# Ushio/MassiveVoxelRayTracing

Measured on AMD Instinct MI355X. Metric: Mrays/sec (primary+secondary) at 1920x1080, 64 spp, higher is better.
Workload: dtype f32; 1 GPU; xyzrgb_dragon stand-in 2048^3 SVO (procedural, pinned by tests/test_scenes.py), wavefront path trace 1920x1080, 183 steps of 16 spp rendered as 64-spp frames (frame buffer cleared + device synchronised per frame), 8 bounces + IBL shadow rays; voxels=18903401, dag_nodes=643656, triangles=1102122, parallelism=1 GPU, device= (gfx950:sramecc+:xnack-, 256 CUs)

## Files before the change

massivevoxelraytracing_amd/csrc/kernels_rt.hip:

```cpp
#include <stdlib.h>

#include <type_traits>

#include "launch.h"
#include "traverse_stream.h"

#define WAVE 64
#define CBLOCK 256

MVRT_DI uint32_t laneId() { return __builtin_amdgcn_mbcnt_hi( ~0u, __builtin_amdgcn_mbcnt_lo( ~0u, 0u ) ); }

MVRT_DI unsigned long long waveSum( unsigned long long v )
{
	for( int o = 32; o > 0; o >>= 1 ) v += __shfl_down( v, o, WAVE );
	return v;
}

static int numCUs();

#define STREAM_WAVES_PER_CU 32

struct BatchIO
{
	const float *rox, *roy, *roz, *rdx, *rdy, *rdz;
// ... 421 lines not shown

template <class T>
MVRT_DI const __attribute__( ( address_space( 4 ) ) ) T* opaquePtr( const T* p )
{
	asm volatile( "" : "+s"( p ) );
	return (const __attribute__( ( address_space( 4 ) ) ) T*)p;
}

struct PtIO
{
	const PtBuffers* table;
	int setIdx;
	uint32_t n;
	int shadowKind;
	int useHint;
	MVRT_UTIL_COUNTERS
	uint32_t dNormal, dShadow, nHits;
	MVRT_DI int kindOf( uint32_t r, uint32_t* i ) const
	{
		const uint32_t kindSlot = ( r >= n ? 1u : 0u ) + ( r >= 2u * n ? 1u : 0u );
		*i = r - ( kindSlot == 0u ? 0u : ( kindSlot == 1u ? n : 2u * n ) );
		return kindSlot == 0 ? 0 : ( kindSlot == 1 ? ( shadowKind ? 1 : 2 ) : 2 );
	}
	MVRT_DI bool load( uint32_t r, f3* ro, f3* rd, uint32_t* hint ) const
	{
		const __attribute__( ( address_space( 4 ) ) ) PtBuffers& buf = *opaquePtr( table );
		const __attribute__( ( address_space( 4 ) ) ) PathSet& in = buf.set[setIdx];
		uint32_t i;
		const int kind = kindOf( r, &i );
		*ro = mk3( in.rox[i], in.roy[i], in.roz[i] );
		if( useHint ) *hint = in.org[i];
		const float *x0 = in.rdx, *y0 = in.rdy, *z0 = in.rdz, *x1 = buf.sx, *y1 = buf.sy, *z1 = buf.sz, *x2 = buf.ex, *y2 = buf.ey, *z2 = buf.ez;
		const float* const px = kind == 0 ? x0 : ( kind == 1 ? x1 : x2 );
		const float* const py = kind == 0 ? y0 : ( kind == 1 ? y1 : y2 );
		const float* const pz = kind == 0 ? z0 : ( kind == 1 ? z1 : z2 );
		*rd = mk3( px[i], py[i], pz[i] );
		return kind == 1;
	}
	MVRT_DI void store( uint32_t r, const StreamHit& h, bool )
	{
		const __attribute__( ( address_space( 4 ) ) ) PtBuffers& buf = *opaquePtr( table );
		uint32_t i;
		const int kind = kindOf( r, &i );
		const bool isHit = h.t != MVRT_MAXF;
		if( kind == 0 )
		{
			buf.hitT[i] = h.t;
			buf.hitPath[i] = h.path;
			buf.hitN[i] = (uint8_t)h.nMajor;
			if( isHit ) atomicAdd( &buf.blockCount[i / CBLOCK], 1u );
		}
		else if( kind == 1 )
		{
			buf.hitS[i] = isHit ? 1 : 0;
		}
		else
		{
			buf.hitE[i] = isHit ? 1 : 0;
			buf.hitEPath[i] = h.path;
		}
		dShadow += kind == 1 ? h.descents : 0u;
		dNormal += kind == 1 ? 0u : h.descents;
		nHits += ( kind != 1 && isHit ) ? 1u : 0u;
	}
};
template <int FL>
__global__ void __launch_bounds__( 64, MVRT_WAVES_OF( FL ) ) kPtTraceStream( PtParams P, TraceWorkspace ws, int stage, int setIdx, int nKinds, int shadowKind, uint32_t chunk,
																			uint32_t raysPerLane, uint32_t minWaves )
{
	PtIO io;
	io.table = P.buf.selfDev;
	io.setIdx = setIdx;
	io.n = P.buf.liveCount[stage];
	io.shadowKind = shadowKind;
	io.useHint = ( FL == 0 && stage > 0 && P.useHints ) ? 1 : 0;
	io.dNormal = io.dShadow = io.nHits = 0;
	const uint64_t total = (uint64_t)io.n * nKinds;
	uint64_t nWaves = gridDim.x;
	if( raysPerLane )
	{
		uint64_t wantWaves = total / ( 64ull * raysPerLane ) + 1;
		if( wantWaves < minWaves ) wantWaves = minWaves;
		if( blockIdx.x >= wantWaves ) return;
		if( wantWaves < nWaves ) nWaves = wantWaves;
	}
	uint64_t c = total / ( nWaves * 4 );
	c = ( c + 63 ) / 64 * 64;
	if( c < 64 ) c = 64;
	if( c > chunk ) c = chunk;
	traceStream<FL>( makeTraceCore( P.svo ), io, total, P.buf.cursors + stage, (uint32_t)c, ws );
	unsigned long long dN = waveSum( (unsigned long long)io.dNormal ), dS = waveSum( (unsigned long long)io.dShadow ), nH = waveSum( (unsigned long long)io.nHits );
#ifdef MVRT_UTIL_STATS
	if( threadIdx.x == 0 )
	{
		atomicAdd( &P.buf.stats[8 + 0], io.utilIters );
		atomicAdd( &P.buf.stats[8 + 1], io.utilActive );
		atomicAdd( &P.buf.stats[8 + 2], io.utilTailIters );
		atomicAdd( &P.buf.stats[8 + 3], io.utilTailActive );
		atomicAdd( &P.buf.stats[12], io.utilRefillClocks );
		atomicAdd( &P.buf.stats[13], io.utilTotalClocks );
		atomicMax( &P.buf.stats[16 + stage], io.utilTailIters );
		atomicAdd( &P.buf.stats[32 + stage], 1ull );
	}
	{
		unsigned long long m = io.utilMaxRayIters;
		for( int o = 32; o > 0; o >>= 1 )
		{
			const unsigned long long t = __shfl_xor( m, o );
			m = t > m ? t : m;
		}
		if( threadIdx.x == 0 ) atomicMax( &P.buf.stats[48 + stage], m );
	}
#endif
	if( threadIdx.x == 0 )
	{
		if( dN ) atomicAdd( &P.buf.stats[2], dN );
		if( dS ) atomicAdd( &P.buf.stats[3], dS );
		if( nH ) atomicAdd( &P.buf.stats[4], nH );
	}
}

MVRT_DI f3 hdriSampleNearest( const HdriDev& h, f3 d, bool isPrimary )
{
	int w = isPrimary ? h.widthPrimary : h.width;
	int hh = isPrimary ? h.heightPrimary : h.height;
	float phi = mvrt_atan2( d.z, d.x ) + MVRT_PI;
	float theta = mvrt_atan2( sqrtf( d.x * d.x + d.z * d.z ), d.y );
	float u = phi / ( MVRT_PI * 2.0f );
	float v = theta / MVRT_PI;
	int x = (int)smin( smax( u * w, 0.0f ), (float)( w - 1.0f ) );
	int y = (int)smin( smax( v * hh, 0.0f ), (float)( hh - 1.0f ) );
	uint64_t index = (uint64_t)y * w + x;
	const float4* px = ( isPrimary && h.pixelsPrimary ) ? h.pixelsPrimary : h.pixels;
	if( !px ) return mk3( 0.0f, 0.0f, 0.0f );
	float4 c = px[index];
	return mk3( c.x, c.y, c.z ) * h.scale;
}
MVRT_DI uint32_t satH( const HdriDev& h, const uint32_t* s, uint32_t x ) { return x == 0 ? 0u : s[h.width * ( h.height - 1 ) + x - 1]; }
MVRT_DI uint32_t satV( const HdriDev& h, const uint32_t* s, uint32_t x, uint32_t y )
{
	if( y == 0 ) return 0u;
	uint32_t s0 = x == 0 ? 0u : s[h.width * ( y - 1 ) + ( x - 1 )];
	uint32_t s1 = s[h.width * ( y - 1 ) + x];
	return s1 - s0;
}
MVRT_DI uint32_t satCount( const HdriDev& h, const uint32_t* s, uint32_t x, uint32_t y )
{
	uint32_t a = ( x == 0 || y == 0 ) ? 0u : s[h.width * ( y - 1 ) + ( x - 1 )];
	uint32_t b = ( y == 0 ) ? 0u : s[h.width * ( y - 1 ) + x];
	uint32_t c = ( x == 0 ) ? 0u : s[h.width * y + ( x - 1 )];
	uint32_t d = s[h.width * y + x];
	return ( d - b ) + ( a - c );
}
MVRT_DI void hdriImportanceSample( const HdriDev& h, f3* dir, f3* L, float* pdf, f3 N, float u0, float u1, float u2, float u3 )
{
	const uint32_t* s = h.sat;
	uint32_t zero = h.zeroTables;
	const float k = 0.8f;
	if( k < N.x ) s = h.sats[0], zero >>= 1;
	else if( N.x < -k ) s = h.sats[1], zero >>= 2;
	else if( k < N.y ) s = h.sats[2], zero >>= 3;
	else if( N.y < -k ) s = h.sats[3], zero >>= 4;
	else if( k < N.z ) s = h.sats[4], zero >>= 5;
	else if( N.z < -k ) s = h.sats[5], zero >>= 6;
	if( zero & 1u )
	{
		*dir = N;
		*L = mk3( 0.0f, 0.0f, 0.0f );
		*pdf = 1.0f;
		return;
	}

	int i = 0, j = h.width;
	while( i < j )
	{
		int m = ( i + j ) / 2;
		float value = (float)satH( h, s, m ) / 4294967296.0f;
		if( value <= u0 ) i = m + 1;
		else j = m;
	}
	uint32_t X = (uint32_t)( i - 1 );
	uint32_t vol = satH( h, s, X + 1 ) - satH( h, s, X );
	i = 0;
	j = h.height;
	while( i < j )
	{
		int m = ( i + j ) / 2;
		float value = (float)satV( h, s, X, m ) / (float)vol;
		if( value <= u1 ) i = m + 1;
		else j = m;
	}
	uint32_t Y = (uint32_t)( i - 1 );
	float pSelection = (float)satCount( h, s, X, Y ) / 4294967296.0f;
	float dTheta = MVRT_PI / (float)h.height;
	float dPhi = 2.0f * MVRT_PI / (float)h.width;
	float theta = Y * dTheta;
	float dH = 2.0f * mvrt_sin( dTheta * 0.5f ) * mvrt_sin( dTheta * 0.5f + theta );
	float sr = dH * dPhi;
	float sY = mixf( mvrt_cos( theta ), mvrt_cos( theta + dTheta ), u2 );
	float phi = dPhi * ( (float)X + u3 ) + MVRT_PI;
	float sX, sZ;
	mvrt_sincos( phi, &sZ, &sX );
	float sinTheta = sqrtf( smax( 1.0f - sY * sY, 0.0f ) );
	*dir = mk3( sX * sinTheta, sY, sZ * sinTheta );
	*pdf = pSelection / sr;
	float4 color = h.pixels[Y * h.width + X];
	*L = mk3( color.x, color.y, color.z ) * h.scale;
}

MVRT_DI f3 sampleLambertian( float a, float b, f3 Ng )
{
	float r = sqrtf( a );
	float theta = b * MVRT_PI * 2.0f;
	float sn, cs;
	mvrt_sincos( theta, &sn, &cs );
	float x = r * cs;
	float y = r * sn;
	float z = sqrtf( smax( 1.0f - a, 0.0f ) );
	const float sign = copysignf( 1.0f, Ng.z );
	const float aa = -1.0f / ( sign + Ng.z );
	const float bb = Ng.x * Ng.y * aa;
	f3 xaxis = mk3( 1.0f + sign * Ng.x * Ng.x * aa, sign * bb, -sign * Ng.x );
	f3 yaxis = mk3( bb, sign + Ng.y * Ng.y * aa, -Ng.y );
	return xaxis * x + yaxis * y + Ng * z;
}

MVRT_DI f3 voxelEmission( const SvoDev& s, uint32_t vIndex, bool withScale )
{
	return rawReflectance( s.attrs[vIndex].y ) * ( withScale ? s.emissionScale : 1.0f );
}

#ifndef MVRT_SHADE_WAVES
#define MVRT_SHADE_WAVES 5
#endif
template <int WAVES, class... ACTIVE>
__global__ void __launch_bounds__( WAVE, WAVES ) kPtShade( PtParams P, int stage, int inSet, ACTIVE... active )
{
	const uint64_t n = P.buf.liveCount[stage];
	const PathSet& in = P.buf.set[inSet];
	const PathSet& out = P.buf.set[inSet ^ 1];
	const bool lastStage = stage >= MVRT_MAX_DEPTH;
	const uint64_t nBlocks = ( n + CBLOCK - 1 ) / CBLOCK;
	for( uint64_t vb = blockIdx.x; vb < nBlocks; vb += gridDim.x )
	{
		uint32_t blockOffset = 0;
		if( !lastStage )
		{
			blockOffset = scanOffset( P.buf.blockCount, P.buf.tileBase, vb );
			if( threadIdx.x == 0 ) P.buf.blockCount[vb] = 0u;
		}
#pragma unroll 1
		for( uint64_t i = vb * CBLOCK + threadIdx.x; i < vb * CBLOCK + CBLOCK; i += WAVE )
		{
			if( i - threadIdx.x >= n ) break;
			const bool valid = i < n;
			bool alive = false;
			uint32_t task = 0, vIndex = 0;
			uint2 attr = make_uint2( 0u, 0u );
			uint64_t hitPath = 0;
			int nMajor = 0;
			float t = MVRT_MAXF;
			f3 ro, rd, T, L;
			if( valid )
			{
				task = in.task[i];
				ro = mk3( in.rox[i], in.roy[i], in.roz[i] );
				rd = mk3( in.rdx[i], in.rdy[i], in.rdz[i] );
				t = P.buf.hitT[i];
				nMajor = P.buf.hitN[i];
				const bool hit = t != MVRT_MAXF;
				hitPath = hit ? P.buf.hitPath[i] : 0ull;
				vIndex = hit ? voxelIndexFromPath( P.svo, hitPath ) : 0u;
				if( hit ) attr = P.svo.attrs[vIndex];
				if( stage == 0 )
				{
					T = mk3( 1.0f, 1.0f, 1.0f );
					L = mk3( 0.0f, 0.0f, 0.0f );
					if( !hit )
					{
						L = L + T * hdriSampleNearest( P.hdri, rd, true );
					}
					else
					{
						L = L + T * rawReflectance( attr.y );
					}
				}
				else
				{
					T = mk3( in.Tx[i], in.Ty[i], in.Tz[i] );
					L = mk3( in.Lx[i], in.Ly[i], in.Lz[i] );
					if( P.hdriEnabled && P.buf.hitS[i] == 0 )
					{
						L = L + mk3( in.nx[i], in.ny[i], in.nz[i] );
					}
					if( stage == 1 && P.extraSamples )
					{
						if( P.buf.hitE[i] )
						{
							const uint32_t ev = voxelIndexFromPath( P.svo, P.buf.hitEPath[i] );
							f3 Le = voxelEmission( P.svo, ev, true );
							L = L + T * Le / (float)( 1 + P.extraSamples );
						}
					}
					if( hit )
					{
						f3 Le = rawReflectance( attr.y ) * P.svo.emissionScale;
						L = L + T * Le * ( stage == 1 ? 1.0f / (float)( 1 + P.extraSamples ) : 1.0f );
					}
				}
				alive = hit && !lastStage;
				if( !alive )
				{
					P.buf.Lsx[task] = L.x;
					P.buf.Lsy[task] = L.y;
					P.buf.Lsz[task] = L.z;
				}
			}
			if( lastStage ) continue;
			const unsigned long long aliveLanes = __ballot( alive );
			const uint32_t rank = __popcll( aliveLanes & ( ( 1ull << threadIdx.x ) - 1ull ) );
			const uint32_t slotBase = blockOffset;
			blockOffset += __popcll( aliveLanes );
			if( alive )
			{
				const uint64_t j = (uint64_t)slotBase + rank;
				uint32_t step, localPixel, localSpp;
				decodeTask( P.frame, task, &step, &localPixel, &localSpp );
				const uint32_t spp = ( P.frame.iteration + step ) * MVRT_SPP_PER_STEP + localSpp;
				const uint32_t stream = hashCombine2( 0u, globalPixel( P.frame, slotPixel( localPixel, active... ) ) );
				int dim = dimBase( stage, P.hdriEnabled, P.extraSamples );
				const f3 R = rawReflectance( attr.x );
				const f3 hitN = getHitN( nMajor, rd );
				const f3 hitP = ro + rd * t;
				f3 nee = mk3( 0.0f, 0.0f, 0.0f );
				if( P.hdriEnabled )
				{
					f2 u01 = pmjSample2d( P.pmj, spp, dim++, stream );
					f2 u23 = pmjSample2d( P.pmj, spp, dim++, stream );
					f3 sdir, emissive;
					float p;
					hdriImportanceSample( P.hdri, &sdir, &emissive, &p, hitN, u01.x, u01.y, u23.x, u23.y );
					nee = T * ( R / MVRT_PI ) * smax( dot3( hitN, sdir ), 0.0f ) * emissive / p;
					P.buf.sx[j] = sdir.x;
					P.buf.sy[j] = sdir.y;
					P.buf.sz[j] = sdir.z;
				}
				T = T * R;
				if( stage == 0 && P.extraSamples )
				{
					f2 u = pmjSample2d( P.pmj, spp, dim++, stream );
					f3 edir = sampleLambertian( u.x, u.y, hitN );
					P.buf.ex[j] = edir.x;
					P.buf.ey[j] = edir.y;
					P.buf.ez[j] = edir.z;
				}
				f2 u = pmjSample2d( P.pmj, spp, dim++, stream );
				f3 bdir = sampleLambertian( u.x, u.y, hitN );
				out.task[j] = task;
				if( P.svo.embedded ) out.org[j] = hintFromVoxelPath( hitPath, P.svo.levels );
				out.rox[j] = hitP.x;
				out.roy[j] = hitP.y;
				out.roz[j] = hitP.z;
				out.rdx[j] = bdir.x;
				out.rdy[j] = bdir.y;
				out.rdz[j] = bdir.z;
				out.Tx[j] = T.x;
				out.Ty[j] = T.y;
				out.Tz[j] = T.z;
				out.Lx[j] = L.x;
				out.Ly[j] = L.y;
				out.Lz[j] = L.z;
				out.nx[j] = nee.x;
				out.ny[j] = nee.y;
				out.nz[j] = nee.z;
			}
		}
	}
}

template <class... ACTIVE>
__global__ void __launch_bounds__( 256 ) kPtAccumulate( PtParams P, float4* __restrict__ fb, ACTIVE... active )
{
	const uint64_t n = P.frame.validOwnedPixels;
	for( uint64_t p = (uint64_t)blockIdx.x * 256 + threadIdx.x; p < n; p += (uint64_t)gridDim.x * 256 )
	{
		const uint64_t px = sizeof...( ACTIVE ) ? (uint64_t)slotPixel( (uint32_t)p, active... ) : p;
		float4 v = fb[px];
		for( int b = 0; b < P.frame.nSteps; b++ )
		{
			const uint64_t base = ( (uint64_t)b * n + p ) * MVRT_SPP_PER_STEP;
			const float4* sx = (const float4*)( P.buf.Lsx + base );
			const float4* sy = (const float4*)( P.buf.Lsy + base );
			const float4* sz = (const float4*)( P.buf.Lsz + base );
			float ax = 0.0f, ay = 0.0f, az = 0.0f;
#pragma unroll
			for( int q = 0; q < MVRT_SPP_PER_STEP / 4; q++ )
			{
				float4 vx = sx[q], vy = sy[q], vz = sz[q];
				ax += vx.x; ax += vx.y; ax += vx.z; ax += vx.w;
				ay += vy.x; ay += vy.y; ay += vy.z; ay += vy.w;
				az += vz.x; az += vz.y; az += vz.z; az += vz.w;
			}
			v.x += ax;
			v.y += ay;
			v.z += az;
			v.w += (float)MVRT_SPP_PER_STEP;
		}
		fb[px] = v;
	}
}

struct AovRecords
{
	const float* hitT;
	const uint64_t* hitPath;
	const uint8_t* hitN;
	const float *rdx, *rdy, *rdz;
};
__global__ void __launch_bounds__( 256 ) kPtAovReduce( SvoDev svo, AovRecords r, uint64_t nPixelSteps, float4* __restrict__ partA, float4* __restrict__ partN )
{
	const uint32_t q = threadIdx.x & 3u;
	for( uint64_t ps = ( (uint64_t)blockIdx.x * 256 + threadIdx.x ) >> 2; ps < nPixelSteps; ps += (uint64_t)gridDim.x * 64 )
	{
		const uint64_t base = ps * MVRT_SPP_PER_STEP + q * 4u;
		const float4 t4 = *(const float4*)( r.hitT + base );
		const ulonglong2 p01 = *(const ulonglong2*)( r.hitPath + base ), p23 = *(const ulonglong2*)( r.hitPath + base + 2 );
		const uint32_t n4 = *(const uint32_t*)( r.hitN + base );
		const float4 dx = *(const float4*)( r.rdx + base ), dy = *(const float4*)( r.rdy + base ), dz = *(const float4*)( r.rdz + base );
		const float t[4] = { t4.x, t4.y, t4.z, t4.w };
		const uint64_t path[4] = { p01.x, p01.y, p23.x, p23.y };
		const float rx[4] = { dx.x, dx.y, dx.z, dx.w }, ry[4] = { dy.x, dy.y, dy.z, dy.w }, rz[4] = { dz.x, dz.y, dz.z, dz.w };
		uint32_t colour[4];
#pragma unroll
		for( int k = 0; k < 4; k++ ) colour[k] = t[k] != MVRT_MAXF ? svo.attrs[voxelIndexFromPath( svo, path[k] )].x : 0u;
		float acc[8] = { 0.0f, 0.0f, 0.0f, 0.0f, 0.0f, 0.0f, 0.0f, 0.0f };
#pragma unroll
		for( uint32_t turn = 0; turn < 4; turn++ )
		{
			if( q == turn )
			{
#pragma unroll
				for( int k = 0; k < 4; k++ )
				{
					if( t[k] == MVRT_MAXF ) continue;
					const f3 a = rawReflectance( colour[k] );
					const f3 n = getHitN( (int)( ( n4 >> ( 8 * k ) ) & 0xFFu ), mk3( rx[k], ry[k], rz[k] ) );
					acc[0] += a.x;
					acc[1] += a.y;
					acc[2] += a.z;
					acc[3] += 1.0f;
					acc[4] += n.x;
					acc[5] += n.y;
					acc[6] += n.z;
					acc[7] += t[k];
				}
			}
#pragma unroll
			for( int j = 0; j < 8; j++ ) acc[j] = __shfl( acc[j], (int)( ( threadIdx.x & 60u ) | turn ) );
		}
		if( q == 0 ) partA[ps] = make_float4( acc[0], acc[1], acc[2], acc[3] );
		if( q == 1 ) partN[ps] = make_float4( acc[4], acc[5], acc[6], acc[7] );
	}
}
template <class... ACTIVE>
__global__ void __launch_bounds__( 256 ) kPtAovAccumulate( uint64_t validOwnedPixels, int nSteps, const float4* __restrict__ partA, const float4* __restrict__ partN,
															 float4* __restrict__ albedo, float4* __restrict__ normalDepth, ACTIVE... active )
{
	for( uint64_t p = (uint64_t)blockIdx.x * 256 + threadIdx.x; p < validOwnedPixels; p += (uint64_t)gridDim.x * 256 )
	{
		const uint64_t px = sizeof...( ACTIVE ) ? (uint64_t)slotPixel( (uint32_t)p, active... ) : p;
		float4 a = albedo[px], n = normalDepth[px];
		for( int b = 0; b < nSteps; b++ )
		{
			const float4 pa = partA[(uint64_t)b * validOwnedPixels + p], pn = partN[(uint64_t)b * validOwnedPixels + p];
			a.x += pa.x; a.y += pa.y; a.z += pa.z; a.w += pa.w;
			n.x += pn.x; n.y += pn.y; n.z += pn.z; n.w += pn.w;
		}
		albedo[px] = a;
		normalDepth[px] = n;
	}
}

struct PtTraceGrid
{
	int grid;
	uint32_t smallRpl, smallMinW;
};
static PtTraceGrid ptTraceGrid( uint64_t rays, int nCUs, int stage, int traceGridDiv )
{
	static const int envDiv = (int)mvrtKnob( "MVRT_TRACE_GRID_DIV", 0 );
	static const int divMaxStage = (int)mvrtKnob( "MVRT_TRACE_DIV_MAX_STAGE", 99 );
	static const uint32_t envRpl = (uint32_t)mvrtKnob( "MVRT_SMALL_RPL", 16 );
	static const uint32_t envMinW = (uint32_t)mvrtKnob( "MVRT_SMALL_MINW", 2048 );
	static const int wpc = (int)mvrtKnob( "MVRT_TRACE_WAVES_PER_CU", 0 );
	int g = streamGrid( rays, nCUs );
	const int div = stage > divMaxStage ? 1 : ( envDiv > 0 ? envDiv : traceGridDiv );
	if( div > 1 && g > nCUs * STREAM_WAVES_PER_CU / div ) g = nCUs * STREAM_WAVES_PER_CU / div;
	if( wpc > 0 && g > nCUs * wpc / ( div > 1 ? div : 1 ) ) g = nCUs * wpc / ( div > 1 ? div : 1 );
	return { g, envRpl, envMinW };
}

static bool shadeDense8( int stage )
{
	static const int dense = (int)mvrtKnob( "MVRT_SHADE8_STAGES", 3 );
	return ( ( dense >> stage ) & 1 ) != 0;
}
static int shadeWavesPerCU( bool dense8 )
{
	static const int bpc8 = (int)mvrtKnob( "MVRT_SHADE_BPC8", 8 ), bpc5 = (int)mvrtKnob( "MVRT_SHADE_BPC5", 5 );
	return ( dense8 ? bpc8 : bpc5 ) * ( CBLOCK / WAVE );
}

static void launchMaskedGenerate( int grid, hipStream_t stream, const PtParams& P, const uint32_t* active );
static void launchMaskedShade( bool dense8, int grid, hipStream_t stream, const PtParams& P, int stage, int setIdx, const uint32_t* active );
static void launchMaskedAccumulate( int grid, hipStream_t stream, const PtParams& P, float4* frameBuffer, const AovBuffers* aov, const uint32_t* active );

int launchPtStep( const SvoDev& svo, const TraceWorkspace& ws, const HdriDev& hdri, const float2* pmj, const CameraPinhole* cams, const PtFrame& frame,
				  const PtBuffers& buf, float4* frameBuffer, int nCUs, PtProfiler* prof, hipStream_t stream, hipEvent_t accumulateAfter, const AovBuffers* aov, float4* moments,
				  const uint32_t* active )
{
	PtParams P;
	P.svo = svo;
	P.hdri = hdri;
	P.pmj = pmj;
	for( int b = 0; b < MVRT_MAX_BATCH; b++ ) P.cams[b] = cams[b < frame.nSteps ? b : 0];
	P.frame = frame;
	P.buf = buf;
	P.hdriEnabled = ( 0.0f < hdri.scale ) ? 1 : 0;
	P.extraSamples = svo.hasEmission ? 1 : 0;
	P.useHints = frame.useHints;
	if( nCUs <= 0 ) nCUs = numCUs();

	const uint64_t nSamples = frame.validOwnedPixels * MVRT_SPP_PER_STEP * frame.nSteps;
	if( nSamples == 0 ) return 0;
	if( nSamples * 3 >= 0xFFFFFFFFull )
	{
		mvrtSetError( "batch too large: %llu samples (ray indices are 32-bit)", (unsigned long long)nSamples );
		return 1;
	}
	if( nSamples > buf.cap )
	{
		mvrtSetError( "path buffers too small: %llu samples > capacity %llu", (unsigned long long)nSamples, (unsigned long long)buf.cap );
		return 1;
	}
	if( !ws.spill )
	{
		mvrtSetError( "internal: traversal workspace missing" );
		return 1;
	}

#define PROF_BEGIN( c ) if( prof ) prof->begin( c, stream )
#define PROF_END() if( prof ) prof->end( stream )

	PROF_BEGIN( MVRT_K_OTHER );
	if( active ) launchMaskedGenerate( persistentGrid( nSamples, 256, nCUs, 8 ), stream, P, active );
	else hipLaunchKernelGGL( kPtGenerate<>, dim3( persistentGrid( nSamples, 256, nCUs, 8 ) ), dim3( 256 ), 0, stream, P );
	PROF_END();

	for( int stage = 0; stage <= MVRT_MAX_DEPTH; stage++ )
	{
		const int setIdx = stage & 1;
		const int shadowKind = ( stage > 0 && P.hdriEnabled ) ? 1 : 0;
		const int extraKind = ( stage == 1 && P.extraSamples ) ? 1 : 0;
		const int nKinds = 1 + shadowKind + extraKind;
		PROF_BEGIN( MVRT_K_TRACE );
		{
			const PtTraceGrid tg = ptTraceGrid( nSamples * nKinds, nCUs, stage, frame.traceGridDiv );
			withFlavour( svo, [&]( auto fl ) {
				hipLaunchKernelGGL( kPtTraceStream<decltype( fl )::value>, dim3( tg.grid ), dim3( 64 ), 0, stream, P, ws, stage, setIdx, nKinds, shadowKind, streamChunk( nSamples * nKinds, tg.grid ),
									tg.smallRpl, tg.smallMinW );
			} );
		}
		PROF_END();
		if( aov && stage == 0 )
		{
			const AovRecords rec = { buf.hitT, buf.hitPath, buf.hitN, buf.set[0].rdx, buf.set[0].rdy, buf.set[0].rdz };
			const uint64_t nPixelSteps = frame.validOwnedPixels * frame.nSteps;
			PROF_BEGIN( MVRT_K_OTHER );
			hipLaunchKernelGGL( kPtAovReduce, dim3( persistentGrid( nPixelSteps * 4, 256, nCUs, 8 ) ), dim3( 256 ), 0, stream, svo, rec, nPixelSteps, aov->partA, aov->partN );
			PROF_END();
		}
		PROF_BEGIN( MVRT_K_OTHER );
		launchScan( buf.blockCount, buf.tileBase, nSamples, (const uint32_t*)( buf.liveCount + stage ), stage < MVRT_MAX_DEPTH ? buf.liveCount + stage + 1 : (uint32_t*)nullptr, buf.stats,
					nKinds, shadowKind, stream );
		PROF_END();
		PROF_BEGIN( MVRT_K_SHADE );
		{
			const bool dense8 = shadeDense8( stage );
			const int wpc = shadeWavesPerCU( dense8 );
			if( active ) launchMaskedShade( dense8, persistentGrid( nSamples, CBLOCK, nCUs, wpc ), stream, P, stage, setIdx, active );
			else if( dense8 )
				hipLaunchKernelGGL( kPtShade<8>, dim3( persistentGrid( nSamples, CBLOCK, nCUs, wpc ) ), dim3( WAVE ), 0, stream, P, stage, setIdx );
			else
				hipLaunchKernelGGL( kPtShade<MVRT_SHADE_WAVES>, dim3( persistentGrid( nSamples, CBLOCK, nCUs, wpc ) ), dim3( WAVE ), 0, stream, P, stage, setIdx );
		}
		PROF_END();
		if( buf.dbgTasks && stage < MVRT_MAX_DEPTH )
			MVRT_HIP( hipMemcpyAsync( buf.dbgTasks + (uint64_t)stage * buf.cap, buf.set[setIdx ^ 1].task, nSamples * 4, hipMemcpyDeviceToDevice, stream ) );
	}
	if( accumulateAfter ) MVRT_HIP( hipStreamWaitEvent( stream, accumulateAfter, 0 ) );
	PROF_BEGIN( MVRT_K_OTHER );
	if( active ) launchMaskedAccumulate( persistentGrid( frame.validOwnedPixels, 256, nCUs, 8 ), stream, P, frameBuffer, nullptr, active );
	else hipLaunchKernelGGL( kPtAccumulate<>, dim3( persistentGrid( frame.validOwnedPixels, 256, nCUs, 8 ) ), dim3( 256 ), 0, stream, P, frameBuffer );
	PROF_END();
	if( aov )
	{
		PROF_BEGIN( MVRT_K_OTHER );
		if( active ) launchMaskedAccumulate( persistentGrid( frame.validOwnedPixels, 256, nCUs, 8 ), stream, P, nullptr, aov, active );
		else
			hipLaunchKernelGGL( kPtAovAccumulate<>, dim3( persistentGrid( frame.validOwnedPixels, 256, nCUs, 8 ) ), dim3( 256 ), 0, stream, frame.validOwnedPixels, frame.nSteps, aov->partA,
								aov->partN, aov->albedo, aov->normalDepth );
		PROF_END();
	}
	if( moments )
	{
		PROF_BEGIN( MVRT_K_OTHER );
		const int rc = launchPtMoments( buf, frame.validOwnedPixels, frame.nSteps, moments, nCUs, stream, active );
		PROF_END();
		if( rc ) return rc;
	}
	MVRT_HIP( hipGetLastError() );
	return 0;
}

static void launchMaskedGenerate( int grid, hipStream_t stream, const PtParams& P, const uint32_t* active )
{
	hipLaunchKernelGGL( kPtGenerate<const uint32_t*>, dim3( grid ), dim3( 256 ), 0, stream, P, active );
}
static void launchMaskedShade( bool dense8, int grid, hipStream_t stream, const PtParams& P, int stage, int setIdx, const uint32_t* active )
{
	if( dense8 ) hipLaunchKernelGGL( ( kPtShade<8, const uint32_t*> ), dim3( grid ), dim3( WAVE ), 0, stream, P, stage, setIdx, active );
	else hipLaunchKernelGGL( ( kPtShade<MVRT_SHADE_WAVES, const uint32_t*> ), dim3( grid ), dim3( WAVE ), 0, stream, P, stage, setIdx, active );
}
static void launchMaskedAccumulate( int grid, hipStream_t stream, const PtParams& P, float4* frameBuffer, const AovBuffers* aov, const uint32_t* active )
{
	if( frameBuffer ) hipLaunchKernelGGL( kPtAccumulate<const uint32_t*>, dim3( grid ), dim3( 256 ), 0, stream, P, frameBuffer, active );
	if( aov )
		hipLaunchKernelGGL( kPtAovAccumulate<const uint32_t*>, dim3( grid ), dim3( 256 ), 0, stream, P.frame.validOwnedPixels, P.frame.nSteps, aov->partA, aov->partN, aov->albedo,
							aov->normalDepth, active );
}
```

massivevoxelraytracing_amd/csrc/mvrt_common.h:

```cpp
#pragma once

#include <hip/hip_runtime.h>
#include <stdint.h>

#include "../../include/mvrt_detmath.h"

#define MVRT_HDI __host__ __device__ __forceinline__
#define MVRT_DI __device__ __forceinline__

#define MVRT_MAXF 3.402823466e+38F
#define MVRT_LEAF 0xFFFFFFFFu
#define MVRT_SPP_PER_STEP 16
#define MVRT_MAX_DEPTH 8
#define MVRT_TILE_PIXELS 256

struct f3
{
	float x, y, z;
};
MVRT_HDI f3 mk3( float x, float y, float z ) { return f3{ x, y, z }; }
MVRT_HDI f3 operator+( f3 a, f3 b ) { return f3{ a.x + b.x, a.y + b.y, a.z + b.z }; }
MVRT_HDI f3 operator-( f3 a, f3 b ) { return f3{ a.x - b.x, a.y - b.y, a.z - b.z }; }
MVRT_HDI f3 operator*( f3 a, f3 b ) { return f3{ a.x * b.x, a.y * b.y, a.z * b.z }; }
MVRT_HDI f3 operator*( f3 a, float b ) { return f3{ a.x * b, a.y * b, a.z * b }; }
// ... 48 lines not shown
	x = ( x ^ ( x >> 16 ) ) & 0x1f00000000ffffull;
	x = ( x ^ ( x >> 32 ) ) & 0x1fffffull;
	return (uint32_t)x;
}
MVRT_HDI void mortonDecode( uint64_t code, uint32_t& x, uint32_t& y, uint32_t& z )
{
	x = compactBy3( code );
	y = compactBy3( code >> 1 );
	z = compactBy3( code >> 2 );
}

MVRT_HDI uint64_t lowerBound( const uint64_t* __restrict__ a, uint64_t lo, uint64_t hi, uint64_t key )
{
	while( lo < hi )
	{
		const uint64_t mid = ( lo + hi ) >> 1;
		if( a[mid] < key ) lo = mid + 1;
		else hi = mid;
	}
	return lo;
}
MVRT_HDI uint32_t popcount8( uint32_t v )
{
	v = ( v & 0x55u ) + ( ( v >> 1 ) & 0x55u );
	v = ( v & 0x33u ) + ( ( v >> 2 ) & 0x33u );
	return ( v & 0x0Fu ) + ( v >> 4 );
}

#define MVRT_PMJ_LENGTH 4096
#define MVRT_PMJ_NSEQ 128
MVRT_HDI uint32_t laineKarras( uint32_t x, uint32_t seed )
{
	x += seed;
	x ^= x * 0x6c50b47cu;
	x ^= x * 0xb82f1e52u;
	x ^= x * 0xc7afe638u;
	x ^= x * 0x8d22f6e6u;
	return x;
}
MVRT_HDI uint32_t reverseBits32( uint32_t v )
{
#if defined( __HIP_DEVICE_COMPILE__ )
	return __brev( v );
#else
	v = ( ( v >> 1 ) & 0x55555555u ) | ( ( v & 0x55555555u ) << 1 );
	v = ( ( v >> 2 ) & 0x33333333u ) | ( ( v & 0x33333333u ) << 2 );
	v = ( ( v >> 4 ) & 0x0F0F0F0Fu ) | ( ( v & 0x0F0F0F0Fu ) << 4 );
	v = ( ( v >> 8 ) & 0x00FF00FFu ) | ( ( v & 0x00FF00FFu ) << 8 );
	return ( v >> 16 ) | ( v << 16 );
#endif
}
MVRT_HDI uint32_t nestedUniformScramble( uint32_t x, uint32_t seed ) { return reverseBits32( laineKarras( reverseBits32( x ), seed ) ); }
MVRT_HDI float scrambleF32( float x, uint32_t seed )
{
	x += 1.0f;
	uint32_t bits = mvrt_f2u( x );
	uint32_t s = 0x3f800000u | ( nestedUniformScramble( bits & 0x7FFFFFu, seed ) & 0x7FFFFFu );
	return mvrt_u2f( s ) - 1.0f;
}
struct f2
{
	float x, y;
};
MVRT_DI f2 pmjSample2d( const float2* __restrict__ table, uint32_t sampleIdx, uint32_t dimension, uint32_t stream )
{
	sampleIdx = nestedUniformScramble( sampleIdx, hashCombine3( stream, dimension, 31082745u ) ) & ( MVRT_PMJ_LENGTH - 1 );
	dimension = nestedUniformScramble( dimension, hashCombine2( stream, 54761983u ) ) & ( MVRT_PMJ_NSEQ - 1 );
	float2 v = table[dimension * MVRT_PMJ_LENGTH + sampleIdx];
	f2 r;
	r.x = scrambleF32( v.x, hashCombine3( stream, dimension, 83927105u ) );
	r.y = scrambleF32( v.y, hashCombine3( stream, dimension, 12654890u ) );
	return r;
}

struct CameraPinhole
{
	f3 o, front, up, right;
	float tanHthetaY, lensR, focus;
};
static_assert( sizeof( CameraPinhole ) == 60, "CameraPinhole must match the reference's 60-byte layout" );

MVRT_HDI void cameraShoot( const CameraPinhole& c, f3* ro, f3* rd, int x, int y, float xo, float yo, int W, int H )
{
	float xf = ( x + xo ) / W;
	float yf = ( y + yo ) / H;
	f3 d = c.right * mixf( -c.tanHthetaY, c.tanHthetaY, xf ) * (float)W / (float)H + c.up * mixf( c.tanHthetaY, -c.tanHthetaY, yf ) + c.front;
	*ro = c.o;
	*rd = d;
}
MVRT_HDI void cameraShootThinLens( const CameraPinhole& c, f3* ro, f3* rd, int x, int y, float xo, float yo, int W, int H, float u0, float u1 )
{
	float xf = ( x + xo ) / W;
	float yf = ( y + yo ) / H;
	f3 focalP = mk3( c.focus * mixf( -c.tanHthetaY, c.tanHthetaY, xf ) * (float)W / (float)H, c.focus * mixf( c.tanHthetaY, -c.tanHthetaY, yf ), c.focus );
	f3 lensP = mk3( mixf( -c.lensR, c.lensR, u0 ), mixf( -c.lensR, c.lensR, u1 ), 0.0f );
	f3 dir = focalP - lensP;
	*rd = c.right * dir.x + c.up * dir.y + c.front * dir.z;
	*ro = c.o + c.right * lensP.x + c.up * lensP.y + c.front * lensP.z;
}

struct alignas( 64 ) Node64
{
	uint32_t children[8];
	uint32_t psum[8];
};
struct SvoDev
{
	const Node64* nodes;
	const uint8_t* masks;
	const uint32_t* psumCold;
	const uint2* attrs;
	uint32_t nNodes, nVoxels;
	f3 lower, upper;
	float dps, emissionScale;
	uint32_t hasEmission;
	uint32_t embedded;
	uint32_t levels;
	uint32_t rootIndex;
	uint32_t rootMask;
	const uint32_t* kids;
	const uint2* topTable;
	uint32_t topLevels;
	uint32_t tree, treeRoot;
	const uint32_t* cellBlocks;
	const uint2* cellEntries;
	uint32_t cellBits;
	uint32_t leafPsumIsPopcount;
};

MVRT_DI f3 getHitN( int major, f3 rd )
{
	f3 n = mk3( 0.0f, 0.0f, 0.0f );
	if( major == 0 ) n.z = 0.0f < rd.z ? -1.0f : 1.0f;
	else if( major == 1 ) n.x = 0.0f < rd.x ? -1.0f : 1.0f;
	else if( major == 2 ) n.y = 0.0f < rd.y ? -1.0f : 1.0f;
	return n;
}
MVRT_DI f3 rawReflectance( uint32_t rgba8 )
{
	return mk3( (float)( rgba8 & 0xFF ) / 255.0f, (float)( ( rgba8 >> 8 ) & 0xFF ) / 255.0f, (float)( ( rgba8 >> 16 ) & 0xFF ) / 255.0f );
}

struct HdriDev
{
	const float4* pixels;
	const float4* pixelsPrimary;
	const uint32_t* sat;
	const uint32_t* sats[6];
	int width, height, widthPrimary, heightPrimary;
	float scale;
	uint32_t zeroTables;
};

void mvrtSetError( const char* fmt, ... );
#define MVRT_HIP( expr )                                                                              \
	do                                                                                                \
	{                                                                                                 \
		hipError_t e_ = ( expr );                                                                     \
		if( e_ != hipSuccess )                                                                        \
		{                                                                                             \
			mvrtSetError( "%s failed: %s (%s:%d)", #expr, hipGetErrorString( e_ ), __FILE__, __LINE__ ); \
			return 1;                                                                                 \
		}                                                                                             \
	} while( 0 )

#ifdef MVRT_EXPERIMENT
#include <stdlib.h>
static inline long long mvrtKnob( const char* name, long long settled ) { const char* e = getenv( name ); return e ? atoll( e ) : settled; }
#else
static inline long long mvrtKnob( const char*, long long settled ) { return settled; }
#endif

static inline uint32_t divUp( uint64_t a, uint64_t b ) { return (uint32_t)( ( a + b - 1 ) / b ); }

struct TraceWorkspace
{
	uint4* spill;
	uint64_t spillStride;
	unsigned long long* cursor;
	uint64_t* paths;
	uint64_t pathCap;
	uint32_t* spillMask;
	uint32_t* spillMask2;
};
```

Measured before the change: 7296 Mrays/s.

## Replace float-divide HDRI binary search with integer thresholds; read shade params from kernarg

The HDRI importance-sampling binary searches now compare raw integer SAT values against a precomputed integer threshold instead of converting and dividing in float every iteration. Helper routines reproduce the exact float comparison semantics at the threshold. The shade kernel gets a slimmer ShadeParams struct that is read directly through the kernarg segment pointer, so it is not copied into registers or scratch. dTheta, dPhi and 1/(1+extra) are precomputed on the host. The risk is subtle off-by-one differences in threshold rounding, plus extra code complexity.

```diff
diff --git a/massivevoxelraytracing_amd/csrc/kernels_rt.hip b/massivevoxelraytracing_amd/csrc/kernels_rt.hip
--- a/massivevoxelraytracing_amd/csrc/kernels_rt.hip
+++ b/massivevoxelraytracing_amd/csrc/kernels_rt.hip
@@ -597,7 +597,7 @@
 	uint32_t d = s[h.width * y + x];
 	return ( d - b ) + ( a - c );
 }
-MVRT_DI void hdriImportanceSample( const HdriDev& h, f3* dir, f3* L, float* pdf, f3 N, float u0, float u1, float u2, float u3 )
+MVRT_DI void hdriImportanceSample( const HdriDev& h, float dTheta, float dPhi, f3* dir, f3* L, float* pdf, f3 N, float u0, float u1, float u2, float u3 )
 {
 	const uint32_t* s = h.sat;
 	uint32_t zero = h.zeroTables;
@@ -616,29 +616,28 @@
 		return;
 	}
 
-	int i = 0, j = h.width;
+	uint32_t last;
+	bool hold = mvrtSatThresholdPow32( u0, &last );
+	int i = 0, j = hold ? h.width : 0;
 	while( i < j )
 	{
 		int m = ( i + j ) / 2;
-		float value = (float)satH( h, s, m ) / 4294967296.0f;
-		if( value <= u0 ) i = m + 1;
+		if( satH( h, s, m ) <= last ) i = m + 1;
 		else j = m;
 	}
 	uint32_t X = (uint32_t)( i - 1 );
 	uint32_t vol = satH( h, s, X + 1 ) - satH( h, s, X );
+	hold = mvrtSatThreshold( (float)vol, u1, &last );
 	i = 0;
-	j = h.height;
+	j = hold ? h.height : 0;
 	while( i < j )
 	{
 		int m = ( i + j ) / 2;
-		float value = (float)satV( h, s, X, m ) / (float)vol;
-		if( value <= u1 ) i = m + 1;
+		if( satV( h, s, X, m ) <= last ) i = m + 1;
 		else j = m;
 	}
 	uint32_t Y = (uint32_t)( i - 1 );
 	float pSelection = (float)satCount( h, s, X, Y ) / 4294967296.0f;
-	float dTheta = MVRT_PI / (float)h.height;
-	float dPhi = 2.0f * MVRT_PI / (float)h.width;
 	float theta = Y * dTheta;
 	float dH = 2.0f * mvrt_sin( dTheta * 0.5f ) * mvrt_sin( dTheta * 0.5f + theta );
 	float sr = dH * dPhi;
@@ -678,12 +677,35 @@
 #ifndef MVRT_SHADE_WAVES
 #define MVRT_SHADE_WAVES 5
 #endif
+struct ShadeParams
+{
+	SvoDev svo;
+	HdriDev hdri;
+	const float2* pmj;
+	PtFrame frame;
+	PtBuffers buf;
+	int hdriEnabled;
+	int extraSamples;
+	float dTheta;
+	float dPhi;
+	float invExtra;
+};
+#define MVRT_AS4 __attribute__( ( address_space( 4 ) ) )
+MVRT_DI const MVRT_AS4 ShadeParams& shadeArgs()
+{
+	const MVRT_AS4 ShadeParams* p = (const MVRT_AS4 ShadeParams*)__builtin_amdgcn_kernarg_segment_ptr();
+	asm volatile( "" : "+s"( p ) );
+	return *p;
+}
+template <class T>
+MVRT_DI const T& genericRef( const MVRT_AS4 T& r )
+{
+	return *(const T*)&r;
+}
 template <int WAVES, class... ACTIVE>
-__global__ void __launch_bounds__( WAVE, WAVES ) kPtShade( PtParams P, int stage, int inSet, ACTIVE... active )
-{
-	const uint64_t n = P.buf.liveCount[stage];
-	const PathSet& in = P.buf.set[inSet];
-	const PathSet& out = P.buf.set[inSet ^ 1];
+__global__ void __launch_bounds__( WAVE, WAVES ) kPtShade( ShadeParams , int stage, int inSet, ACTIVE... active )
+{
+	const uint64_t n = shadeArgs().buf.liveCount[stage];
 	const bool lastStage = stage >= MVRT_MAX_DEPTH;
 	const uint64_t nBlocks = ( n + CBLOCK - 1 ) / CBLOCK;
 	for( uint64_t vb = blockIdx.x; vb < nBlocks; vb += gridDim.x )
@@ -691,8 +713,10 @@
 		uint32_t blockOffset = 0;
 		if( !lastStage )
 		{
-			blockOffset = scanOffset( P.buf.blockCount, P.buf.tileBase, vb );
-			if( threadIdx.x == 0 ) P.buf.blockCount[vb] = 0u;
+			const MVRT_AS4 PtBuffers& buf = shadeArgs().buf;
+			uint32_t* const blockCount = buf.blockCount;
+			blockOffset = scanOffset( blockCount, buf.tileBase, vb );
+			if( threadIdx.x == 0 ) blockCount[vb] = 0u;
 		}
 #pragma unroll 1
 		for( uint64_t i = vb * CBLOCK + threadIdx.x; i < vb * CBLOCK + CBLOCK; i += WAVE )
@@ -708,22 +732,27 @@
 			f3 ro, rd, T, L;
 			if( valid )
 			{
+				const MVRT_AS4 ShadeParams& P = shadeArgs();
+				const MVRT_AS4 PtBuffers& buf = P.buf;
+				const MVRT_AS4 PathSet& in = buf.set[inSet];
+				const SvoDev& svo = genericRef( P.svo );
+				const int hdriEnabled = P.hdriEnabled, extraSamples = P.extraSamples;
 				task = in.task[i];
 				ro = mk3( in.rox[i], in.roy[i], in.roz[i] );
 				rd = mk3( in.rdx[i], in.rdy[i], in.rdz[i] );
-				t = P.buf.hitT[i];
-				nMajor = P.buf.hitN[i];
+				t = buf.hitT[i];
+				nMajor = buf.hitN[i];
 				const bool hit = t != MVRT_MAXF;
-				hitPath = hit ? P.buf.hitPath[i] : 0ull;
-				vIndex = hit ? voxelIndexFromPath( P.svo, hitPath ) : 0u;
-				if( hit ) attr = P.svo.attrs[vIndex];
+				hitPath = hit ? buf.hitPath[i] : 0ull;
+				vIndex = hit ? voxelIndexFromPath( svo, hitPath ) : 0u;
+				if( hit ) attr = svo.attrs[vIndex];
 				if( stage == 0 )
 				{
 					T = mk3( 1.0f, 1.0f, 1.0f );
 					L = mk3( 0.0f, 0.0f, 0.0f );
 					if( !hit )
 					{
-						L = L + T * hdriSampleNearest( P.hdri, rd, true );
+						L = L + T * hdriSampleNearest( genericRef( P.hdri ), rd, true );
 					}
 					else
 					{
@@ -734,31 +763,32 @@
 				{
 					T = mk3( in.Tx[i], in.Ty[i], in.Tz[i] );
 					L = mk3( in.Lx[i], in.Ly[i], in.Lz[i] );
-					if( P.hdriEnabled && P.buf.hitS[i] == 0 )
+					if( hdriEnabled && buf.hitS[i] == 0 )
 					{
 						L = L + mk3( in.nx[i], in.ny[i], in.nz[i] );
 					}
-					if( stage == 1 && P.extraSamples )
+					const float invExtra = P.invExtra;
+					if( stage == 1 && extraSamples )
 					{
-						if( P.buf.hitE[i] )
+						if( buf.hitE[i] )
 						{
-							const uint32_t ev = voxelIndexFromPath( P.svo, P.buf.hitEPath[i] );
-							f3 Le = voxelEmission( P.svo, ev, true );
-							L = L + T * Le / (float)( 1 + P.extraSamples );
+							const uint32_t ev = voxelIndexFromPath( svo, buf.hitEPath[i] );
+							f3 Le = voxelEmission( svo, ev, true );
+							L = L + T * Le * invExtra;
 						}
 					}
 					if( hit )
 					{
-						f3 Le = rawReflectance( attr.y ) * P.svo.emissionScale;
-						L = L + T * Le * ( stage == 1 ? 1.0f / (float)( 1 + P.extraSamples ) : 1.0f );
+						f3 Le = rawReflectance( attr.y ) * svo.emissionScale;
+						L = L + T * Le * ( stage == 1 ? invExtra : 1.0f );
 					}
 				}
 				alive = hit && !lastStage;
 				if( !alive )
 				{
-					P.buf.Lsx[task] = L.x;
-					P.buf.Lsy[task] = L.y;
-					P.buf.Lsz[task] = L.z;
+					buf.Lsx[task] = L.x;
+					buf.Lsy[task] = L.y;
+					buf.Lsz[task] = L.z;
 				}
 			}
 			if( lastStage ) continue;
@@ -769,38 +799,48 @@
 			if( alive )
 			{
 				const uint64_t j = (uint64_t)slotBase + rank;
-				uint32_t step, localPixel, localSpp;
-				decodeTask( P.frame, task, &step, &localPixel, &localSpp );
-				const uint32_t spp = ( P.frame.iteration + step ) * MVRT_SPP_PER_STEP + localSpp;
-				const uint32_t stream = hashCombine2( 0u, globalPixel( P.frame, slotPixel( localPixel, active... ) ) );
-				int dim = dimBase( stage, P.hdriEnabled, P.extraSamples );
+				f3 nee = mk3( 0.0f, 0.0f, 0.0f );
+				f3 bdir;
 				const f3 R = rawReflectance( attr.x );
 				const f3 hitN = getHitN( nMajor, rd );
 				const f3 hitP = ro + rd * t;
-				f3 nee = mk3( 0.0f, 0.0f, 0.0f );
-				if( P.hdriEnabled )
 				{
-					f2 u01 = pmjSample2d( P.pmj, spp, dim++, stream );
-					f2 u23 = pmjSample2d( P.pmj, spp, dim++, stream );
-					f3 sdir, emissive;
-					float p;
-					hdriImportanceSample( P.hdri, &sdir, &emissive, &p, hitN, u01.x, u01.y, u23.x, u23.y );
-					nee = T * ( R / MVRT_PI ) * smax( dot3( hitN, sdir ), 0.0f ) * emissive / p;
-					P.buf.sx[j] = sdir.x;
-					P.buf.sy[j] = sdir.y;
-					P.buf.sz[j] = sdir.z;
+					const MVRT_AS4 ShadeParams& P = shadeArgs();
+					const MVRT_AS4 PtBuffers& buf = P.buf;
+					const int hdriEnabled = P.hdriEnabled, extraSamples = P.extraSamples;
+					const float2* const pmj = P.pmj;
+					const PtFrame& frame = genericRef( P.frame );
+					uint32_t step, localPixel, localSpp;
+					decodeTask( frame, task, &step, &localPixel, &localSpp );
+					const uint32_t spp = ( frame.iteration + step ) * MVRT_SPP_PER_STEP + localSpp;
+					const uint32_t stream = hashCombine2( 0u, globalPixel( frame, slotPixel( localPixel, active... ) ) );
+					int dim = dimBase( stage, hdriEnabled, extraSamples );
+					if( hdriEnabled )
+					{
+						f2 u01 = pmjSample2d( pmj, spp, dim++, stream );
+						f2 u23 = pmjSample2d( pmj, spp, dim++, stream );
+						f3 sdir, emissive;
+						float p;
+						hdriImportanceSample( genericRef( P.hdri ), P.dTheta, P.dPhi, &sdir, &emissive, &p, hitN, u01.x, u01.y, u23.x, u23.y );
+						nee = T * ( R / MVRT_PI ) * smax( dot3( hitN, sdir ), 0.0f ) * emissive / p;
+						buf.sx[j] = sdir.x;
+						buf.sy[j] = sdir.y;
+						buf.sz[j] = sdir.z;
+					}
+					T = T * R;
+					if( stage == 0 && extraSamples )
+					{
+						f2 u = pmjSample2d( pmj, spp, dim++, stream );
+						f3 edir = sampleLambertian( u.x, u.y, hitN );
+						buf.ex[j] = edir.x;
+						buf.ey[j] = edir.y;
+						buf.ez[j] = edir.z;
+					}
+					f2 u = pmjSample2d( pmj, spp, dim++, stream );
+					bdir = sampleLambertian( u.x, u.y, hitN );
 				}
-				T = T * R;
-				if( stage == 0 && P.extraSamples )
-				{
-					f2 u = pmjSample2d( P.pmj, spp, dim++, stream );
-					f3 edir = sampleLambertian( u.x, u.y, hitN );
-					P.buf.ex[j] = edir.x;
-					P.buf.ey[j] = edir.y;
-					P.buf.ez[j] = edir.z;
-				}
-				f2 u = pmjSample2d( P.pmj, spp, dim++, stream );
-				f3 bdir = sampleLambertian( u.x, u.y, hitN );
+				const MVRT_AS4 ShadeParams& P = shadeArgs();
+				const MVRT_AS4 PathSet& out = P.buf.set[inSet ^ 1];
 				out.task[j] = task;
 				if( P.svo.embedded ) out.org[j] = hintFromVoxelPath( hitPath, P.svo.levels );
 				out.rox[j] = hitP.x;
@@ -957,7 +997,7 @@
 }
 
 static void launchMaskedGenerate( int grid, hipStream_t stream, const PtParams& P, const uint32_t* active );
-static void launchMaskedShade( bool dense8, int grid, hipStream_t stream, const PtParams& P, int stage, int setIdx, const uint32_t* active );
+static void launchMaskedShade( bool dense8, int grid, hipStream_t stream, const ShadeParams& S, int stage, int setIdx, const uint32_t* active );
 static void launchMaskedAccumulate( int grid, hipStream_t stream, const PtParams& P, float4* frameBuffer, const AovBuffers* aov, const uint32_t* active );
 
 int launchPtStep( const SvoDev& svo, const TraceWorkspace& ws, const HdriDev& hdri, const float2* pmj, const CameraPinhole* cams, const PtFrame& frame,
@@ -974,6 +1014,17 @@
 	P.hdriEnabled = ( 0.0f < hdri.scale ) ? 1 : 0;
 	P.extraSamples = svo.hasEmission ? 1 : 0;
 	P.useHints = frame.useHints;
+	ShadeParams S;
+	S.svo = svo;
+	S.hdri = hdri;
+	S.pmj = pmj;
+	S.frame = frame;
+	S.buf = buf;
+	S.hdriEnabled = P.hdriEnabled;
+	S.extraSamples = P.extraSamples;
+	S.dTheta = MVRT_PI / (float)hdri.height;
+	S.dPhi = 2.0f * MVRT_PI / (float)hdri.width;
+	S.invExtra = 1.0f / (float)( 1 + P.extraSamples );
 	if( nCUs <= 0 ) nCUs = numCUs();
 
 	const uint64_t nSamples = frame.validOwnedPixels * MVRT_SPP_PER_STEP * frame.nSteps;
@@ -1033,11 +1084,11 @@
 		{
 			const bool dense8 = shadeDense8( stage );
 			const int wpc = shadeWavesPerCU( dense8 );
-			if( active ) launchMaskedShade( dense8, persistentGrid( nSamples, CBLOCK, nCUs, wpc ), stream, P, stage, setIdx, active );
+			if( active ) launchMaskedShade( dense8, persistentGrid( nSamples, CBLOCK, nCUs, wpc ), stream, S, stage, setIdx, active );
 			else if( dense8 )
-				hipLaunchKernelGGL( kPtShade<8>, dim3( persistentGrid( nSamples, CBLOCK, nCUs, wpc ) ), dim3( WAVE ), 0, stream, P, stage, setIdx );
+				hipLaunchKernelGGL( kPtShade<8>, dim3( persistentGrid( nSamples, CBLOCK, nCUs, wpc ) ), dim3( WAVE ), 0, stream, S, stage, setIdx );
 			else
-				hipLaunchKernelGGL( kPtShade<MVRT_SHADE_WAVES>, dim3( persistentGrid( nSamples, CBLOCK, nCUs, wpc ) ), dim3( WAVE ), 0, stream, P, stage, setIdx );
+				hipLaunchKernelGGL( kPtShade<MVRT_SHADE_WAVES>, dim3( persistentGrid( nSamples, CBLOCK, nCUs, wpc ) ), dim3( WAVE ), 0, stream, S, stage, setIdx );
 		}
 		PROF_END();
 		if( buf.dbgTasks && stage < MVRT_MAX_DEPTH )
@@ -1072,10 +1123,10 @@
 {
 	hipLaunchKernelGGL( kPtGenerate<const uint32_t*>, dim3( grid ), dim3( 256 ), 0, stream, P, active );
 }
-static void launchMaskedShade( bool dense8, int grid, hipStream_t stream, const PtParams& P, int stage, int setIdx, const uint32_t* active )
-{
-	if( dense8 ) hipLaunchKernelGGL( ( kPtShade<8, const uint32_t*> ), dim3( grid ), dim3( WAVE ), 0, stream, P, stage, setIdx, active );
-	else hipLaunchKernelGGL( ( kPtShade<MVRT_SHADE_WAVES, const uint32_t*> ), dim3( grid ), dim3( WAVE ), 0, stream, P, stage, setIdx, active );
+static void launchMaskedShade( bool dense8, int grid, hipStream_t stream, const ShadeParams& S, int stage, int setIdx, const uint32_t* active )
+{
+	if( dense8 ) hipLaunchKernelGGL( ( kPtShade<8, const uint32_t*> ), dim3( grid ), dim3( WAVE ), 0, stream, S, stage, setIdx, active );
+	else hipLaunchKernelGGL( ( kPtShade<MVRT_SHADE_WAVES, const uint32_t*> ), dim3( grid ), dim3( WAVE ), 0, stream, S, stage, setIdx, active );
 }
 static void launchMaskedAccumulate( int grid, hipStream_t stream, const PtParams& P, float4* frameBuffer, const AovBuffers* aov, const uint32_t* active )
 {
diff --git a/massivevoxelraytracing_amd/csrc/mvrt_common.h b/massivevoxelraytracing_amd/csrc/mvrt_common.h
--- a/massivevoxelraytracing_amd/csrc/mvrt_common.h
+++ b/massivevoxelraytracing_amd/csrc/mvrt_common.h
@@ -224,6 +224,38 @@
 	uint32_t zeroTables;
 };
 
+MVRT_HDI uint32_t mvrtSatLast( float F )
+{
+	if( F >= 4294967296.0f ) return 0xFFFFFFFFu;
+	if( F < 16777216.0f ) return (uint32_t)F;
+	const uint32_t bits = mvrt_f2u( F ), half = 1u << ( ( bits >> 23 ) - 127u - 24u );
+	return (uint32_t)F + half - ( bits & 1u );
+}
+MVRT_HDI float mvrtSatWhole( float F )
+{
+	F = F < 8388608.0f ? (float)(uint32_t)F : F;
+	return F <= 4294967296.0f ? F : 4294967296.0f;
+}
+MVRT_HDI bool mvrtSatThresholdPow32( float u, uint32_t* last )
+{
+	*last = 0u;
+	if( !( 0.0f <= u ) ) return false;
+	*last = mvrtSatLast( mvrtSatWhole( u * 4294967296.0f ) );
+	return true;
+}
+MVRT_HDI float mvrtSatNextF( float f ) { return f < 16777216.0f ? f + 1.0f : mvrt_u2f( mvrt_f2u( f ) + 1u ); }
+MVRT_HDI float mvrtSatPrevF( float f ) { return f <= 16777216.0f ? f - 1.0f : mvrt_u2f( mvrt_f2u( f ) - 1u ); }
+MVRT_HDI bool mvrtSatThreshold( float v, float u, uint32_t* last )
+{
+	*last = 0u;
+	if( !( 0.0f / v <= u ) ) return false;
+	float F = mvrtSatWhole( u * v );
+	while( F > 0.0f && !( F / v <= u ) ) F = mvrtSatPrevF( F );
+	while( F < 4294967296.0f && mvrtSatNextF( F ) / v <= u ) F = mvrtSatNextF( F );
+	*last = mvrtSatLast( F );
+	return true;
+}
+
 void mvrtSetError( const char* fmt, ... );
 #define MVRT_HIP( expr )                                                                              \
 	do                                                                                                \
```

Measured after the change: 7309 Mrays/s (median of 6 runs). No clear change (+0.2%).
